# bytedance/monolith

Hardware: AMD Instinct MI355X
Metric: embedding lookups+updates/sec at 1B ids x dim64, Zipf(1.2) batch=65536 (higher is better)
Workload: dtype f32

## Files before the change

monolith_amd/_lib.py:

```python
import ctypes as C
import os
import subprocess

_DIR = os.path.dirname(os.path.abspath(__file__))
_SO = os.path.join(_DIR, "libmhte.so")
_SRC = os.path.join(_DIR, "csrc", "mhte.hip")
_DEPS = [_SRC] + sorted(os.path.join(_DIR, "csrc", h) for h in os.listdir(os.path.join(_DIR, "csrc"))
                        if h.endswith(".h")) + [os.path.join(_DIR, "..", "include", "monolith_amd_hash_table.h")]
_OVERRIDE = os.environ.get("MHTE_LIBRARY")

MHTE_OK = 0
MHTE_INVALID_ARGUMENT = 3
MHTE_NOT_FOUND = 5
MHTE_RESOURCE_EXHAUSTED = 8
MHTE_FAILED_PRECONDITION = 9
MHTE_INTERNAL = 13
MHTE_UNAVAILABLE = 14

MHTE_IDS_UNIQUE = 1
MHTE_SUM_DUPLICATES = 2
MHTE_EXACT_ORDER = 1
MHTE_DEFER_SLOWPATH = 2
MHTE_LAYOUT_ONE_FID_UNIQUE_ROWS = 1
ABI_VERSION = 19
# ... 71 lines not shown
def _stale():
  if not os.path.exists(_SO):
    return True
  if os.path.exists(_HASH_FILE):
    with open(_HASH_FILE) as f:
      return f.read().strip() != _source_hash()
  t = os.path.getmtime(_SO)
  return any(os.path.exists(d) and os.path.getmtime(d) > t for d in _DEPS)


def build_library(force=False, verbose=False):
  if not force and not _stale():
    _try_build_eager_loop(verbose)
    return _SO
  cmd = ["hipcc", "--offload-arch=gfx950", "-O3", "-std=c++17", "-ffp-contract=off", "-shared",
         "-fPIC", "-o", _SO, _SRC]
  if verbose:
    print(" ".join(cmd))
  if os.path.exists(_HASH_FILE):
    os.remove(_HASH_FILE)
  src_hash = _source_hash()
  subprocess.check_call(cmd)
  with open(_HASH_FILE, "w") as f:
    f.write(src_hash + "\n")
  _try_build_eager_loop(verbose)
  return _SO


_EAGER_SO = os.path.join(_DIR, "libmhte_eager.so")
_EAGER_SRC = os.path.join(_DIR, "csrc", "eager_loop.c")

# ... 184 lines not shown
```

monolith_amd/csrc/mhte.hip:

```cpp
#include <hip/hip_runtime.h>
#include <hip/hip_ext.h>
#include <hip/hip_fp16.h>

#include <algorithm>
#include <chrono>
#include <cstdio>
#include <cstdlib>
#include <cstring>
#include <memory>
#include <atomic>
#include <exception>
#include <mutex>
#include <future>
#include <thread>
#include <stdexcept>
#include <string>
#include <vector>

#include "../../include/monolith_amd_hash_table.h"
#include <unistd.h>
#include <dirent.h>
#include <ctype.h>

#include "mhte_ckpt.h"
// ... 419 lines not shown
    const uint32_t nb = (un + kDdBlock - 1) / kDdBlock;
    LAUNCH_HOT(kTagDedup, dd_insert_fast_kernel, nb, kDdBlock, st, d, ids, un, uids);
    LAUNCH_HOT(kTagDedup, dd_place_fast_kernel, nb, kDdBlock, st, d, un, inverse, lst_start, lst_end,
               seg_pos);
    const uint32_t nb_rank = (un + 1023) / 1024;
    const uint32_t hgrid = std::min<uint32_t>(256, un / (kLightMax + 1) + 1);
    LAUNCH_HOT(kTagDedup, dd_finish_kernel, nb_rank + hgrid, 1024, st, d, un, nb_rank, inverse,
               lst_start, lst_end, seg_pos, 0, n_unique_dev);
    hipError_t le = hipGetLastError();
    if (le != hipSuccess) {
      clean_cap = 0;
      HIP_OK(le);
    }
  }
};

struct Shape {
  int G;
  int VEC;
};
static Shape pick_shape(uint32_t dim, bool vec_ok) {
  Shape s;
  s.VEC = vec_ok ? 4 : 1;
  uint32_t units = (dim + s.VEC - 1) / s.VEC;
  uint32_t g = 8;
  while (g < units && g < 64) g <<= 1;
  s.G = int(g);
  return s;
}
static inline bool aligned16(const void* p) { return (reinterpret_cast<uintptr_t>(p) & 15u) == 0; }
// ... 572 lines not shown
    const uint32_t others = nxt.nblk + uint32_t(sp.enabled);
    const uint32_t slots = uint32_t(2 * num_cus);
    const uint32_t held = nxt.nblk;
    const uint32_t room = slots > held + 64 ? slots - held : 64u;
    auto blocks_for = [&](int unr) {
      const int64_t groups = (n + unr - 1) / unr;
      return uint32_t((groups * sh.G + kRdBlock - 1) / kRdBlock);
    };
    int unr = 2;
    while (unr < 3 && blocks_for(unr) > 2 * room) ++unr;
    const uint32_t nblk_l = std::min(blocks_for(unr), room);
    const dim3 grid(others + nblk_l);
    TableView v = view;
    v.trace = trace_region(kTagStepFwd, grid.x, kRdBlock);
    const bool basic = basic_opts();
#define CALLU(G_, V_, U_)                                                                        \
  do {                                                                                           \
    if (basic) {                                                                                 \
      LAUNCH_HOT(kTagStepFwd, (step_fwd_kernel<G_, V_, U_, true>), grid, kRdBlock, st, nxt, v, ids, n, out, \
                 count_hits ? 1 : 0, sp, nblk_l);                                                \
    } else {                                                                                     \
      LAUNCH_HOT(kTagStepFwd, (step_fwd_kernel<G_, V_, U_, false>), grid, kRdBlock, st, nxt, v, ids, n, out, \
                 count_hits ? 1 : 0, sp, nblk_l);                                                \
    }                                                                                            \
  } while (0)
#define CALL(G_, V_)                              \
  do {                                            \
    if (unr == 2) { CALLU(G_, V_, 2); }           \
    else { CALLU(G_, V_, 3); }                    \
  } while (0)
    DISPATCH_G_VEC(sh, CALL);
#undef CALL
#undef CALLU
    HIP_OK(hipGetLastError());
  }

  void step_backward(DedupWs& ws, DedupWs* ws_next, const int64_t* uids, int64_t n_max,
                     const uint32_t* n_dev, const float* grads, int64_t n, float* grad_u,
// ... 105 lines not shown
      da.ctr = ahead.ctr;
      da.ids = ahead.ids;
      da.cap_mask = ahead.cap_mask;
      da.n = ahead.n;
      da.nblk = ahead.nblk;
    }
    const dim3 grid(da.nblk + nblk_build + c.nblk_items + c.nblk_ids);
    TableView v = view;
    v.trace = trace_region(kTagStepBwd, grid.x, 256);
    const RunView cur = ws.rv;
    const bool basic = basic_opts();
    static const bool no_optk = getenv("MHTE_NO_OPTK") != nullptr;
    const bool filt = flt_slots != nullptr;
    const int optk =
        (!basic && nseg == 1 && sh.VEC == 4 && !view.seg[0].sr16 && !no_optk && !filt) ? int(view.seg[0].opt) : -1;
#define CALL_FILT(G_, V_, S_, F_)                                                                                \
  LAUNCH_HOT(kTagStepBwd, (step_bwd_kernel<G_, V_, S_, F_, -1, true>), grid, 256, st, nxt, nblk_build, v, cur, c, a, po, da)
#define CALL_OPTK(G_, K_)                                                                                     \
  LAUNCH_HOT(kTagStepBwd, (step_bwd_kernel<G_, 4, true, true, K_>), grid, 256, st, nxt, nblk_build, v, cur, c, a, po, da)
#define CALL(G_, V_) \
  do {                                                                                               \
    if (filt) {                                                                                      \
      if (basic && nseg == 1) CALL_FILT(G_, V_, true, false);                                        \
      else if (basic) CALL_FILT(G_, V_, false, false);                                               \
      else if (nseg == 1) CALL_FILT(G_, V_, true, true);                                             \
      else CALL_FILT(G_, V_, false, true);                                                           \
    } else if (V_ == 4 && optk == kOptMomentum) {                                                    \
      CALL_OPTK(G_, kOptMomentum);                                                                   \
    } else if (V_ == 4 && optk == kOptAdadelta) {                                                    \
      CALL_OPTK(G_, kOptAdadelta);                                                                   \
    } else if (V_ == 4 && optk == kOptRmsprop) {                                                     \
      CALL_OPTK(G_, kOptRmsprop);                                                                    \
    } else if (V_ == 4 && optk == kOptRmspropV2) {                                                   \
      CALL_OPTK(G_, kOptRmspropV2);                                                                  \
    } else if (V_ == 4 && optk == kOptAdam) {                                                        \
      CALL_OPTK(G_, kOptAdam);                                                                       \
    } else if (V_ == 4 && optk == kOptAmsgrad) {                                                     \
      CALL_OPTK(G_, kOptAmsgrad);                                                                    \
    } else if (!basic && nseg == 1) {                                                                \
      LAUNCH_HOT(kTagStepBwd, (step_bwd_kernel<G_, V_, true, true>), grid, 256, st, nxt, nblk_build, v, cur, c, a, po, da); \
    } else if (!basic) {                                                                             \
      LAUNCH_HOT(kTagStepBwd, (step_bwd_kernel<G_, V_, false, true>), grid, 256, st, nxt, nblk_build, v, cur, c, a, po, da); \
    } else if (nseg == 1) {                                                                          \
      LAUNCH_HOT(kTagStepBwd, (step_bwd_kernel<G_, V_, true>), grid, 256, st, nxt, nblk_build, v, cur, c, a, po, da);  \
    } else {                                                                                         \
      LAUNCH_HOT(kTagStepBwd, (step_bwd_kernel<G_, V_, false>), grid, 256, st, nxt, nblk_build, v, cur, c, a, po, da); \
    }                                                                                                \
  } while (0)
    DISPATCH_G_VEC(sh, CALL);
#undef CALL
#undef CALL_OPTK
#undef CALL_FILT
    hipError_t le = hipGetLastError();
    ws.r_stage = 0;
    if (nblk_build) {
      ws_next->r_stage = 2;
      ws_next->r_hints = true;
      ws_next->r_prealloc = reserve_next;
      ws_next->r_res_ctr = view.ctr;
      ws_next->r_res_serial = ctr_serial;
    }
    if (le != hipSuccess) {
      ws.r_clean_cap = 0;
      if (ws_next) ws_next->r_clean_cap = 0;
      HIP_OK(le);
    }
    filter_maintain(st, uint64_t(n));
// ... 3620 lines not shown
```

monolith_amd/csrc/mhte_step_kernels.h:

```cpp
#ifndef MHTE_STEP_KERNELS_H_
#define MHTE_STEP_KERNELS_H_

#include "mhte_kernels.h"

namespace mhte {

constexpr int kRdBlock = 1024;
constexpr int kRdLds = 2048;
constexpr int kRdStride = kRdLds + 1;
constexpr int kRdMaxBlocks = 64;
constexpr int kLongRun = kLightMax;
constexpr int kStepLightMax = 32;
constexpr int kMaxLongRuns = 16;
constexpr uint32_t kItemTarget = 256;
constexpr uint32_t kSpecSlackRows = 32;
#ifndef MHTE_BWD_OCC
#define MHTE_BWD_OCC 5
#endif
constexpr int kBwdBlocksPerCu = MHTE_BWD_OCC;

__device__ __forceinline__ void lds_barrier() {
  asm volatile("s_waitcnt lgkmcnt(0)\n\ts_barrier" ::: "memory");
}
__device__ __forceinline__ void lds_wave_sync() {
  asm volatile("s_waitcnt lgkmcnt(0)" ::: "memory");
}

__device__ __forceinline__ uint32_t run_pack(uint32_t first, uint32_t off, uint32_t cnt) {
  return (first << 21) | (off << 11) | cnt;
}
__device__ __forceinline__ uint32_t run_cnt(uint32_t v) { return v & 0x7ffu; }
__device__ __forceinline__ uint32_t run_off(uint32_t v) { return (v >> 11) & 0x3ffu; }
__device__ __forceinline__ uint32_t run_first(uint32_t v) { return v >> 21; }

// ... 39 lines not shown
  }
  if (i < 4) d.ctr[i] = 0;
}

struct RdLds {
  unsigned long long key[kRdStride];
  uint32_t cnt[kRdStride];
  uint32_t off[kRdStride];
  uint32_t first[kRdStride];
  uint16_t pos[kRdBlock];
  uint32_t wtot[16];
  uint32_t bm[kMaxLongRuns][32];
  uint32_t bmpre[kMaxLongRuns][32];
  uint8_t lslot[kRdStride + 3];
  uint32_t nlong;
};

__device__ __forceinline__ uint32_t rd_home(int64_t id) {
  return uint32_t(hash_key(id) >> 40) & (kRdLds - 1);
}

__device__ __forceinline__ void rd_dedup_role(const RunView& d, uint32_t bid, RdLds& L,
                                              WaveTrace& wt) {
  const uint32_t t = threadIdx.x;
  for (uint32_t i = t; i < uint32_t(kRdStride); i += kRdBlock) {
    L.key[i] = static_cast<unsigned long long>(kEmptyKey);
    L.cnt[i] = 0;
    L.lslot[i] = 0xff;
  }
  if (t < kMaxLongRuns * 32) (&L.bm[0][0])[t] = 0;
  if (t == 0) L.nlong = 0;
  if (bid == 0 && t < 4) d.ctr[t] = 0;
  const uint32_t p = bid * kRdBlock + t;
  const bool valid = p < d.n;
  const int64_t id = valid ? d.ids[p] : 0;
  lds_barrier();
  uint32_t ls = 0, arr = 0;
  if (valid) {
    if (id == kEmptyKey) {
      ls = kRdLds;
    } else {
      ls = rd_home(id);
      for (;;) {
        unsigned long long k = L.key[ls];
        if (k == static_cast<unsigned long long>(kEmptyKey)) {
          k = atomicCAS(&L.key[ls], static_cast<unsigned long long>(kEmptyKey),
                        static_cast<unsigned long long>(id));
          if (k == static_cast<unsigned long long>(kEmptyKey)) break;
        }
        if (k == static_cast<unsigned long long>(id)) break;
// ... 68 lines not shown
    const uint32_t c = L.cnt[ls], o = L.off[ls];
    uint32_t rank = 0;
    if (lsl != 0xffu) {
      rank = L.bmpre[lsl][t >> 5] + __popc(L.bm[lsl][t >> 5] & ((1u << (t & 31u)) - 1u));
    } else if (c > 1) {
      uint32_t i = 0;
      for (; i + 8 <= c; i += 8) {
        uint32_t x[8];
#pragma unroll
        for (int q = 0; q < 8; ++q) x[q] = L.pos[o + i + q];
#pragma unroll
        for (int q = 0; q < 8; ++q) rank += (x[q] < t) ? 1u : 0u;
      }
      for (; i < c; ++i) rank += (uint32_t(L.pos[o + i]) < t) ? 1u : 0u;
    }
    d.seg[bid * kRdBlock + o + rank] = uint16_t(t);
  }
  wt.mark(3);
  uint32_t lbase;
  if (speaker) {
    if (id != kEmptyKey) {
      while (cas_old != kEmptyKey && cas_old != id) {
        gs = (gs + 1u) & d.cap_mask;
        cas_old = static_cast<int64_t>(atomicCAS(reinterpret_cast<unsigned long long*>(&d.hs[gs].key),
                                                 static_cast<unsigned long long>(kEmptyKey),
                                                 static_cast<unsigned long long>(id)));
      }
    }
    lbase = uint32_t(atomicAdd(&d.hs[gs].cp, (static_cast<unsigned long long>(p) << 32) |
                                                 static_cast<unsigned long long>(L.cnt[ls])));
  }
  for (uint32_t i = t; i < uint32_t(kRdStride); i += kRdBlock) {
    d.btab_key[size_t(bid) * kRdStride + i] = static_cast<int64_t>(L.key[i]);
    d.btab_val[size_t(bid) * kRdStride + i] = run_pack(L.first[i] & 0x3ffu, L.off[i] & 0x3ffu, L.cnt[i]);
  }
  if (speaker) {
    const uint32_t c = L.cnt[ls];
    if (lbase + c <= uint32_t(kLightMax)) {
      const uint32_t o = L.off[ls];
      for (uint32_t i = 0; i < c; ++i)
        d.hlist[size_t(gs) * kLightMax + lbase + i] = bid * kRdBlock + uint32_t(L.pos[o + i]);
    }
  }
  wt.mark(4);
}

__global__ __launch_bounds__(kRdBlock) void rd_dedup_kernel(RunView d) {
  __shared__ RdLds L;
  WaveTrace wt(nullptr);
  rd_dedup_role(d, blockIdx.x, L, wt);
}

constexpr int kRd4Threads = 256;
constexpr int kRd4PerThread = kRdBlock / kRd4Threads;
struct __attribute__((aligned(16))) RdLds4 {
  unsigned long long key[kRdStride];
// ... 240 lines not shown
  return uint32_t(m < 0 ? m + int64_t(nshards) : m);
}
struct PackCtl {
  int64_t* send_ids;
  const unsigned long long* peer_win;
  unsigned long long peer_ids_off;
  uint32_t* slot_off;
  uint32_t* flags;
  uint32_t world, ids_block, rows_block;
  uint32_t hdr_word;
  uint32_t cap, id_off, row_off, dim;
};

__device__ __forceinline__ void rd_emit_items(const RunView& d, int64_t id, uint32_t hu, uint32_t c,
                                              uint32_t hrow, uint32_t hspec, unsigned long long hloc,
                                              int lane) {
  const uint32_t val = (uint32_t(lane) < d.nblk) ? rd_find_run_opt(d, uint32_t(lane), id) : 0u;
  const unsigned long long bm = __ballot(val != 0u);
  const uint32_t nbk = rd_item_blocks(c, d.item_target);
  const uint32_t b0 = uint32_t(lane) & ~(nbk - 1u);
  const unsigned long long rmask = (nbk == 64 ? ~0ull : ((1ull << nbk) - 1ull)) << b0;
  const bool leader = (uint32_t(lane) == b0) && (bm & rmask) != 0ull;
  const unsigned long long lm = __ballot(leader);
  const uint32_t nitems = __popcll(lm);
  uint32_t w0 = 0;
  if (lane == 0) w0 = atomicAdd(&d.ctr[2], nitems);
  w0 = __shfl(w0, 0);
  const uint32_t k = __popcll(lm & ((1ull << b0) - 1ull));
  if (leader) {
    ItemHdr hd;
    hd.id = id;
    hd.u = hu;
    hd.meta = b0 | (nbk << 8) | (k << 16) | (nitems << 24);
    hd.row = hrow;
    hd.spec = hspec;
    hd.loc = hloc;
    d.item_hdr[w0 + k] = hd;
  }
  if ((bm & rmask) != 0ull) d.item_runs[size_t(w0 + k) * 64 + (uint32_t(lane) - b0)] = val;
}

constexpr unsigned long long kNoLoc = ~0ull;
struct __attribute__((aligned(16))) URec {
  int64_t id;
  uint32_t cnt;
  uint32_t pos;
  uint32_t slot;
  uint32_t row;
  unsigned long long loc;
};
struct ProbeOut {
  URec* urec;
  uint32_t reserve;
};

template <bool PACK = false, bool PROBE = false>
__device__ __forceinline__ void rd_build_role(const RunView& d, uint32_t light_max, uint32_t bid,
                                              uint32_t nblocks, const PackCtl* pc = nullptr,
                                              const TableView* tv = nullptr, ProbeOut po = ProbeOut{}) {
  constexpr int Q = kBuildSlotsPerLane;
  __shared__ uint32_t sh_tot[4];
  __shared__ uint32_t sh_base;
  __shared__ uint32_t sh_mtot[PROBE ? 4 : 1];
  __shared__ uint32_t sh_mbase;
  __shared__ uint8_t sh_stage[PROBE ? 4 * 256 : 4];
  __shared__ uint32_t sh_pc[PACK ? kMaxShards : 1], sh_pb[PACK ? kMaxShards : 1];
  const uint32_t t = threadIdx.x;
  const int lane = t & 63;
  const uint32_t nslots = d.cap_mask + 2u;
  for (uint32_t bb = bid * (256u * Q); bb < nslots; bb += nblocks * (256u * Q)) {
    const uint32_t base = bb + (t >> 6) * (64u * Q);
    int64_t key[Q];
    uint32_t cnt[Q], pos[Q];
    unsigned long long occ[Q];
// ... 3 lines not shown
      lds_barrier();
    }
#pragma unroll
    for (int q = 0; q < Q; ++q) {
      const uint32_t sl = base + q * 64 + lane;
      const bool in = sl < nslots;
      const RdSlot sv = d.hs[in ? sl : 0u];
      key[q] = in ? sv.key : kEmptyKey;
      cnt[q] = in ? uint32_t(sv.cp) : 0u;
      pos[q] = in ? uint32_t(sv.cp >> 32) : 0u;
    }
#pragma unroll
    for (int q = 0; q < Q; ++q) {
      const uint32_t sl = base + q * 64 + lane;
      const bool o = key[q] != kEmptyKey;
      if (o) {
        d.hs[sl] = RdSlot{kEmptyKey, 0ull};
        if (sl == d.cap_mask + 1u) key[q] = kEmptyKey;
      }
      occ[q] = __ballot(o);
      total += uint32_t(__popcll(occ[q]));
    }
    uint32_t pown[Q], prank[Q];
    if (PACK) {
#pragma unroll
      for (int q = 0; q < Q; ++q) {
        pown[q] = prank[q] = 0;
        if ((occ[q] >> lane) & 1ull) {
          pown[q] = shard_of_id(key[q], pc->world);
          prank[q] = atomicAdd(&sh_pc[pown[q]], 1u);
        }
      }
    }
    if (lane == 0) sh_tot[t >> 6] = total;
// ... 122 lines not shown
          uint32_t m0 = sh_mbase;
          for (uint32_t w2 = 0; w2 < (t >> 6); ++w2) m0 += sh_mtot[w2];
          lds_barrier();
          if (miss) spec = m0 + uint32_t(__popcll(mm & ((1ull << lane) - 1ull)));
        }
        const unsigned long long floc = found ? (((fs & 4) ? i2 : i1) << 2) | uint64_t(fs & 3) : kNoLoc;
        const uint32_t frow = found ? fr : spec;
        if (have) {
          URec rec;
          rec.id = kid;
          rec.cnt = kc;
          rec.pos = kp;
          rec.slot = base + (src >> 6) * 64u + (src & 63u);
          rec.row = frow;
          rec.loc = floc;
          po.urec[kw0 + r] = rec;
        }
        unsigned long long hm = __ballot(have && kc > light_max);
        while (hm) {
          const int s2 = __ffsll(static_cast<long long>(hm)) - 1;
          hm &= hm - 1ull;
          const unsigned long long hl = __shfl(floc, s2);
          rd_emit_items(d, __shfl(kid, s2), kw0 + r0 + uint32_t(s2), __shfl(kc, s2),
                        hl != kNoLoc ? __shfl(frow, s2) : kNoRow, hl != kNoLoc ? kNoRow : __shfl(frow, s2),
                        hl != kNoLoc ? hl : 0ull, lane);
        }
      }
    }
  }
  if (t == 0) {
    if (atomicAdd(&d.ctr[1], 1u) == nblocks - 1) *d.n_unique = atomicAdd(&d.ctr[0], 0u);
  }
}

__global__ __launch_bounds__(256) void rd_build_kernel(RunView d, uint32_t light_max) {
  rd_build_role(d, light_max, blockIdx.x, gridDim.x);
}
__global__ __launch_bounds__(256) void rd_build_probe_kernel(RunView d, uint32_t light_max, TableView tv,
                                                             ProbeOut po) {
  rd_build_role<false, true>(d, light_max, blockIdx.x, gridDim.x, nullptr, &tv, po);
// ... 371 lines not shown
  out.deferred = deferred;
  return out;
}

struct ApplyLds {
  uint32_t pos[(256 / 8) * kStepLightMax];
  uint32_t rstart[65];
  uint32_t rval[64];
  float sum[256 * 4];
  uint32_t last;
};

template <int G, int VEC, bool ONESEG, bool HINT = false, bool FULL = false, int OPTK = -1, int FILT = -1>
__device__ __forceinline__ void rd_apply_role(const TableView& tv, const RunView& d,
                                              const ApplyCtl& c, const ApplyArgs& a, uint32_t bid,
                                              WaveTrace& wt, ApplyLds& L) {
  constexpr int WIN = G < 8 ? G : 8;
  constexpr int NG = 256 / G;
  const int lane = threadIdx.x & 63;
  const int j = lane & (G - 1);
  const int gbase = lane & ~(G - 1);
  const int grp = threadIdx.x / G;
  const uint32_t dim = tv.dim;
  const uint32_t e = uint32_t(j) * VEC;
  const bool ev = e < dim;

  if (bid >= c.nblk_items) {
    const uint32_t stride = c.nblk_ids * uint32_t(NG);
    const uint32_t k = bid - c.nblk_items;
    const uint32_t wave_s = __builtin_amdgcn_readfirstlane(threadIdx.x >> 6);
    uint32_t nu = c.n_max;
// ... 256 lines not shown
  for (uint32_t w = bid;; w += c.nblk_items) {
    const uint32_t nitems_all = d.ctr[2];
    const ItemHdr hd = d.item_hdr[w];
    const uint32_t rval = d.item_runs[size_t(w) * 64 + lane];
    asm volatile("" ::"v"(hd.meta), "v"(rval), "v"(nitems_all));
    if (w >= nitems_all) break;
    wt.mark(0);
    const uint32_t b0 = hd.meta & 0xffu, nbk = (hd.meta >> 8) & 0xffu, kk = (hd.meta >> 16) & 0xffu,
                   nitems = hd.meta >> 24;
    const bool ihint = hd.row != kNoRow;
    GBucket* const hb = global_bucket(tv.buckets + (hd.loc >> 2));
    int64_t vkey = hd.id;
    if (ihint && !c.trusted && threadIdx.x == 0) vkey = hb->key[hd.loc & 3ull];
    Probe<G> pr = probe_issue<G>(tv, hd.id, threadIdx.x < G && !ihint, j);
    const uint32_t reserved = threadIdx.x < G ? hd.spec : kNoRow;
    if (threadIdx.x < 64) {
      const uint32_t val = (uint32_t(lane) < nbk) ? rval : 0u;
      uint32_t incl = run_cnt(val);
#pragma unroll
      for (int o = 1; o < 64; o <<= 1) {
        const uint32_t v = __shfl_up(incl, o);
        if (lane >= o) incl += v;
      }
      sh_rval[lane] = val;
      sh_rstart[lane + 1] = incl;
      if (lane == 0) sh_rstart[0] = 0;
    }
    lds_barrier();
    wt.mark(1);
    const uint32_t E = c.pre_summed ? 0u : sh_rstart[64];
// ... 138 lines not shown
        sr.is_new = false;
        sr.deferred = false;
        if (valid && threadIdx.x == 0) hb->ts[hd.loc & 3ull] = vgpr_copy_of_uniform(a.ts);
      } else {
        sr = upsert_resolve<G>(tv, (Bucket*)pr.b, hd.id, valid, pr.k, pr.row, lane, vgpr_copy_of_uniform(a.ts),
                               reserved);
      }
      if (sr.deferred) {
        uint32_t ed = e;
#ifndef MHTE_NO_ANTIHOIST
        asm volatile("" : "+v"(ed));
#endif
        if (ev) tot.store(c.grad_u + int64_t(hd.u) * dim + ed);
        if (j == 0) defer_id(tv, c.pending, hd.u);
      } else if (valid) {
        if (FULL) optimize_row_reg_full<VEC, ONESEG, OPTK>(tv, row_ptr(tv, sr.r), sr.is_new, e, tot, a);
        else optimize_row_reg<VEC, ONESEG>(tv, row_ptr(tv, sr.r), sr.is_new, e, tot, a);
      }
    }
    wt.mark(4);
    lds_barrier();
  }
}

constexpr int kExactThreads = 512;
constexpr int kExactBufFloats = 16384;
constexpr int kExactMaxRows = 512;
struct __attribute__((aligned(16))) ExactLds {
  float buf[2][kExactBufFloats];
  uint32_t pos[3][kExactMaxRows];
  uint32_t rstart[65];
  uint32_t rbase[64];
// ... 137 lines not shown
__global__ __launch_bounds__(kExactThreads) void rd_exact_sum_kernel(RunView d, const float* __restrict__ grads,
                                                                     uint32_t dim, float* __restrict__ part) {
  __shared__ ExactLds L;
  rd_exact_sum_role<VEC>(d, grads, dim, ExactToPart{part, dim}, blockIdx.x, gridDim.x, L);
}

struct SlowArgs {
  const int64_t* uids;
  const float* grad_u;
  const uint32_t* pending;
  ApplyArgs a;
  int32_t enabled;
};


template <int G, int VEC, int UNR, bool BASIC = true>
__global__ __launch_bounds__(kRdBlock, 8) __attribute__((amdgpu_num_sgpr(80))) void step_fwd_kernel(RunView nxt, TableView tv,
                                                            const int64_t* __restrict__ ids,
                                                            int64_t n, float* __restrict__ out,
                                                            int count_hits, SlowArgs sp,
                                                            uint32_t nblk_l) {
  __shared__ __attribute__((aligned(16))) RdLds L;
  static_assert(sizeof(BfsSlot) * kMaxCuckooCount + sizeof(CuckooRecord) * kMaxBfsPathLen <=
                    sizeof(RdLds), "BFS scratch must fit the dedup's LDS");
  WaveTrace wt(tv.trace);
  uint32_t bid = blockIdx.x;
  if (bid < nxt.nblk) {
    rd_dedup_role(nxt, bid, L, wt);
    wt.end(3u);
    return;
  }
  bid -= nxt.nblk;
  if (sp.enabled) {
    if (bid == 0) {
      if (threadIdx.x < 64) {
        BfsSlot* q = reinterpret_cast<BfsSlot*>(&L);
        CuckooRecord* path = reinterpret_cast<CuckooRecord*>(q + kMaxCuckooCount);
        slowpath_role<VEC, kOpOptimize, false, true, BASIC>(tv, sp.uids, sp.grad_u, nullptr, nullptr, sp.a,
                                                            nullptr, sp.pending, q, path);
      }
      wt.end(4u);
      return;
    }
    bid -= 1;
  }
  const int64_t ngroups = (n + UNR - 1) / UNR;
  const uint32_t lbid = bid;
  const int64_t g_first = (int64_t(lbid) * kRdBlock + threadIdx.x) / G;
  int64_t id_first;
  {
    const int j = int(threadIdx.x & 63u) & (G - 1);
    const int64_t p0 = g_first * UNR + j;
    id_first = ids[(j < UNR && p0 < n) ? p0 : 0];
    if (!(j < UNR && p0 < n)) id_first = 0;
  }
  if (sp.enabled) {
    if (threadIdx.x == 0) {
      if (__hip_atomic_load(&tv.ctr->n_pending, __ATOMIC_RELAXED, __HIP_MEMORY_SCOPE_AGENT) != 0u) {
        while (__hip_atomic_load(&tv.ctr->n_pending, __ATOMIC_RELAXED, __HIP_MEMORY_SCOPE_AGENT) != 0u)
          __builtin_amdgcn_s_sleep(16);
        __builtin_amdgcn_fence(__ATOMIC_ACQUIRE, "agent");
      }
    }
    __syncthreads();
  }
  if (g_first < ngroups) lookup_role_u<G, VEC, UNR, 2>(tv, ids, n, nullptr, out, count_hits, g_first, &id_first);
#pragma unroll 1
  for (int64_t g = g_first + int64_t(nblk_l) * kRdBlock / G; g < ngroups;
       g += int64_t(nblk_l) * kRdBlock / G)
    lookup_role_u<G, VEC, UNR, 2>(tv, ids, n, nullptr, out, count_hits, g);
  wt.end(5u);
}

struct DedupArgs {
  RdSlot* hs;
  uint32_t* hlist;
  int64_t* btab_key;
  uint32_t* btab_val;
  uint16_t* seg;
  uint32_t* ctr;
  const int64_t* ids;
  uint32_t cap_mask, n;
  uint32_t nblk;
};

union __attribute__((aligned(16))) StepBwdLds {
  ApplyLds apply;
  RdLds4 dedup;
};
template <int G, int VEC, bool ONESEG, bool FULL = false, int OPTK = -1, bool FILT = false>
__global__ __launch_bounds__(256, kBwdBlocksPerCu) void step_bwd_kernel(RunView nxt, uint32_t nblk_build,
                                                       TableView tv, RunView cur, ApplyCtl c,
                                                       ApplyArgs a, ProbeOut po, DedupArgs da) {
  __shared__ StepBwdLds L;
  WaveTrace wt(tv.trace);
  uint32_t bid = blockIdx.x;
  if (bid < da.nblk) {
    RunView d{};
    d.hs = da.hs;
    d.hlist = da.hlist;
    d.btab_key = da.btab_key;
    d.btab_val = da.btab_val;
    d.seg = da.seg;
    d.ctr = da.ctr;
    d.ids = da.ids;
    d.cap_mask = da.cap_mask;
    d.n = da.n;
    d.nblk = da.nblk;
    rd_dedup4_role(d, bid, L.dedup);
    wt.end(3u);
    return;
  }
  bid -= da.nblk;
  if (bid < nblk_build) {
    rd_build_role<false, true>(nxt, uint32_t(kStepLightMax), bid, nblk_build, nullptr, &tv, po);
    wt.end(6u);
    return;
  }
  bid -= nblk_build;
  rd_apply_role<G, VEC, ONESEG, false, FULL, OPTK, FILT ? 1 : 0>(tv, cur, c, a, bid, wt, L.apply);
  wt.end(bid < c.nblk_items ? 7u : 8u);
}

struct GatherCtl {
  const float* in;
  float* out;
  const uint32_t* index;
  float* part;
  uint32_t* arrive;
  int64_t n_max;
  uint32_t dim;
  uint32_t nblk_items;
  uint32_t nblk_ids;
  uint32_t index_is_offset;
  const unsigned long long* peer_win;
  unsigned long long peer_out_off;
// ... 305 lines not shown
```

Measured before the change: 4.360 billion.

## Preload hot kernel args, add sc1 vector stores for dedup/build outputs, and prefetch rows

Enables AMDGPU kernel-argument preloading and reorders the fused step kernel signatures so the hot scalars (ids, counts, block splits, switch mask) come first and land in SGPRs. It also replaces scattered scalar stores of dedup directory, segment, hlist, item headers, urec and hash-slot resets with 16-byte global stores using the sc1 cache-policy bit, or relaxed atomic stores. The apply role gains an optional row prefetch into LDS. Each piece sits behind an environment switch, and there are no-preload kernel variants for comparison. The cost is more LDS per block, more code paths, and reliance on inline assembly and a compiler flag.

```diff
diff --git a/monolith_amd/_lib.py b/monolith_amd/_lib.py
--- a/monolith_amd/_lib.py
+++ b/monolith_amd/_lib.py
@@ -109,7 +109,7 @@
     _try_build_eager_loop(verbose)
     return _SO
   cmd = ["hipcc", "--offload-arch=gfx950", "-O3", "-std=c++17", "-ffp-contract=off", "-shared",
-         "-fPIC", "-o", _SO, _SRC]
+         "-fPIC", "-mllvm", "-amdgpu-kernarg-preload-count=16", "-o", _SO, _SRC]
   if verbose:
     print(" ".join(cmd))
   if os.path.exists(_HASH_FILE):
diff --git a/monolith_amd/csrc/mhte.hip b/monolith_amd/csrc/mhte.hip
--- a/monolith_amd/csrc/mhte.hip
+++ b/monolith_amd/csrc/mhte.hip
@@ -457,6 +457,24 @@
     }
   }
 };
+
+constexpr uint32_t kWtDefault = 1u | 2u | 8u | 16u | 32u;
+struct StepSwitches {
+  bool preload;
+  uint32_t sw;
+};
+static const StepSwitches& step_switches() {
+  static const StepSwitches v = [] {
+    StepSwitches r;
+    r.preload = getenv("MHTE_NO_PRELOAD") == nullptr;
+    r.sw = getenv("MHTE_NO_ITEM_PREFETCH") == nullptr ? kSwItemPf : 0u;
+    uint32_t wt = kWtDefault;
+    if (const char* e = getenv("MHTE_WT_STORES")) wt = uint32_t(atoi(e)) & 63u;
+    r.sw |= wt << 8;
+    return r;
+  }();
+  return v;
+}
 
 struct Shape {
   int G;
@@ -1059,14 +1077,25 @@
     TableView v = view;
     v.trace = trace_region(kTagStepFwd, grid.x, kRdBlock);
     const bool basic = basic_opts();
+    const StepSwitches& ss = step_switches();
+    const uint32_t sw = (ss.sw & (kSwWtDir | kSwWtSeg | kSwWtHlist)) | (v.trace ? kSwTrace : 0u);
+    const int32_t spe = sp.enabled;
 #define CALLU(G_, V_, U_)                                                                        \
   do {                                                                                           \
-    if (basic) {                                                                                 \
-      LAUNCH_HOT(kTagStepFwd, (step_fwd_kernel<G_, V_, U_, true>), grid, kRdBlock, st, nxt, v, ids, n, out, \
-                 count_hits ? 1 : 0, sp, nblk_l);                                                \
+    if (!ss.preload) {                                                                           \
+      if (basic) {                                                                               \
+        LAUNCH_HOT(kTagStepFwd, (step_fwd_kernel_np<G_, V_, U_, true>), grid, kRdBlock, st, nxt, ids, n, nxt.ids, \
+                   nxt.n, nxt.nblk, nblk_l, spe, sw, v, out, count_hits ? 1 : 0, sp);            \
+      } else {                                                                                   \
+        LAUNCH_HOT(kTagStepFwd, (step_fwd_kernel_np<G_, V_, U_, false>), grid, kRdBlock, st, nxt, ids, n, nxt.ids, \
+                   nxt.n, nxt.nblk, nblk_l, spe, sw, v, out, count_hits ? 1 : 0, sp);            \
+      }                                                                                          \
+    } else if (basic) {                                                                          \
+      LAUNCH_HOT(kTagStepFwd, (step_fwd_kernel<G_, V_, U_, true>), grid, kRdBlock, st, ids, n, nxt.ids, nxt.n, \
+                 nxt.nblk, nblk_l, spe, sw, nxt, v, out, count_hits ? 1 : 0, sp);                \
     } else {                                                                                     \
-      LAUNCH_HOT(kTagStepFwd, (step_fwd_kernel<G_, V_, U_, false>), grid, kRdBlock, st, nxt, v, ids, n, out, \
-                 count_hits ? 1 : 0, sp, nblk_l);                                                \
+      LAUNCH_HOT(kTagStepFwd, (step_fwd_kernel<G_, V_, U_, false>), grid, kRdBlock, st, ids, n, nxt.ids, nxt.n, \
+                 nxt.nblk, nblk_l, spe, sw, nxt, v, out, count_hits ? 1 : 0, sp);                \
     }                                                                                            \
   } while (0)
 #define CALL(G_, V_)                              \
@@ -1202,10 +1231,14 @@
     const bool filt = flt_slots != nullptr;
     const int optk =
         (!basic && nseg == 1 && sh.VEC == 4 && !view.seg[0].sr16 && !no_optk && !filt) ? int(view.seg[0].opt) : -1;
+    const StepSwitches& ss = step_switches();
+    const uint32_t sw = (ss.sw & (kSwItemPf | kSwWtReset | kSwWtUrec | kSwWtItems)) | (v.trace ? kSwTrace : 0u);
+#define BWD_LEAD cur.ctr, cur.item_hdr, cur.item_runs, c.urec, c.nblk_items, nblk_build, da.nblk, uint32_t(std::min<int64_t>(n_max, 0x7fffffff)), sw
+#define BWD_REST v, cur, c, a, po, da
 #define CALL_FILT(G_, V_, S_, F_)                                                                                \
-  LAUNCH_HOT(kTagStepBwd, (step_bwd_kernel<G_, V_, S_, F_, -1, true>), grid, 256, st, nxt, nblk_build, v, cur, c, a, po, da)
+  LAUNCH_HOT(kTagStepBwd, (step_bwd_kernel<G_, V_, S_, F_, -1, true>), grid, 256, st, BWD_LEAD, nxt, BWD_REST)
 #define CALL_OPTK(G_, K_)                                                                                     \
-  LAUNCH_HOT(kTagStepBwd, (step_bwd_kernel<G_, 4, true, true, K_>), grid, 256, st, nxt, nblk_build, v, cur, c, a, po, da)
+  LAUNCH_HOT(kTagStepBwd, (step_bwd_kernel<G_, 4, true, true, K_>), grid, 256, st, BWD_LEAD, nxt, BWD_REST)
 #define CALL(G_, V_) \
   do {                                                                                               \
     if (filt) {                                                                                      \
@@ -1226,19 +1259,25 @@
     } else if (V_ == 4 && optk == kOptAmsgrad) {                                                     \
       CALL_OPTK(G_, kOptAmsgrad);                                                                    \
     } else if (!basic && nseg == 1) {                                                                \
-      LAUNCH_HOT(kTagStepBwd, (step_bwd_kernel<G_, V_, true, true>), grid, 256, st, nxt, nblk_build, v, cur, c, a, po, da); \
+      LAUNCH_HOT(kTagStepBwd, (step_bwd_kernel<G_, V_, true, true>), grid, 256, st, BWD_LEAD, nxt, BWD_REST); \
     } else if (!basic) {                                                                             \
-      LAUNCH_HOT(kTagStepBwd, (step_bwd_kernel<G_, V_, false, true>), grid, 256, st, nxt, nblk_build, v, cur, c, a, po, da); \
+      LAUNCH_HOT(kTagStepBwd, (step_bwd_kernel<G_, V_, false, true>), grid, 256, st, BWD_LEAD, nxt, BWD_REST); \
+    } else if (!ss.preload && nseg == 1) {                                                           \
+      LAUNCH_HOT(kTagStepBwd, (step_bwd_kernel_np<G_, V_, true>), grid, 256, st, nxt, BWD_LEAD, BWD_REST); \
+    } else if (!ss.preload) {                                                                        \
+      LAUNCH_HOT(kTagStepBwd, (step_bwd_kernel_np<G_, V_, false>), grid, 256, st, nxt, BWD_LEAD, BWD_REST); \
     } else if (nseg == 1) {                                                                          \
-      LAUNCH_HOT(kTagStepBwd, (step_bwd_kernel<G_, V_, true>), grid, 256, st, nxt, nblk_build, v, cur, c, a, po, da);  \
+      LAUNCH_HOT(kTagStepBwd, (step_bwd_kernel<G_, V_, true>), grid, 256, st, BWD_LEAD, nxt, BWD_REST);  \
     } else {                                                                                         \
-      LAUNCH_HOT(kTagStepBwd, (step_bwd_kernel<G_, V_, false>), grid, 256, st, nxt, nblk_build, v, cur, c, a, po, da); \
+      LAUNCH_HOT(kTagStepBwd, (step_bwd_kernel<G_, V_, false>), grid, 256, st, BWD_LEAD, nxt, BWD_REST); \
     }                                                                                                \
   } while (0)
     DISPATCH_G_VEC(sh, CALL);
 #undef CALL
 #undef CALL_OPTK
 #undef CALL_FILT
+#undef BWD_LEAD
+#undef BWD_REST
     hipError_t le = hipGetLastError();
     ws.r_stage = 0;
     if (nblk_build) {
diff --git a/monolith_amd/csrc/mhte_step_kernels.h b/monolith_amd/csrc/mhte_step_kernels.h
--- a/monolith_amd/csrc/mhte_step_kernels.h
+++ b/monolith_amd/csrc/mhte_step_kernels.h
@@ -18,6 +18,20 @@
 #define MHTE_BWD_OCC 5
 #endif
 constexpr int kBwdBlocksPerCu = MHTE_BWD_OCC;
+
+constexpr uint32_t kSwItemPf = 1u;
+constexpr uint32_t kSwTrace = 2u;
+constexpr uint32_t kSwWtDir = 1u << 8;
+constexpr uint32_t kSwWtSeg = 1u << 9;
+constexpr uint32_t kSwWtHlist = 1u << 10;
+constexpr uint32_t kSwWtReset = 1u << 11;
+constexpr uint32_t kSwWtUrec = 1u << 12;
+constexpr uint32_t kSwWtItems = 1u << 13;
+
+typedef unsigned int wt_u32x4 __attribute__((ext_vector_type(4)));
+__device__ __forceinline__ void store_wt16(void* p, wt_u32x4 v) {
+  asm volatile("global_store_dwordx4 %0, %1, off sc1\n\ts_nop 1" ::"v"((MHTE_GLOBAL void*)p), "v"(v) : "memory");
+}
 
 __device__ __forceinline__ void lds_barrier() {
   asm volatile("s_waitcnt lgkmcnt(0)\n\ts_barrier" ::: "memory");
@@ -87,6 +101,7 @@
   uint32_t bmpre[kMaxLongRuns][32];
   uint8_t lslot[kRdStride + 3];
   uint32_t nlong;
+  uint16_t __attribute__((aligned(16))) segout[kRdBlock];
 };
 
 __device__ __forceinline__ uint32_t rd_home(int64_t id) {
@@ -94,7 +109,7 @@
 }
 
 __device__ __forceinline__ void rd_dedup_role(const RunView& d, uint32_t bid, RdLds& L,
-                                              WaveTrace& wt) {
+                                              WaveTrace& wt, uint32_t sw = 0) {
   const uint32_t t = threadIdx.x;
   for (uint32_t i = t; i < uint32_t(kRdStride); i += kRdBlock) {
     L.key[i] = static_cast<unsigned long long>(kEmptyKey);
@@ -103,10 +118,11 @@
   }
   if (t < kMaxLongRuns * 32) (&L.bm[0][0])[t] = 0;
   if (t == 0) L.nlong = 0;
-  if (bid == 0 && t < 4) d.ctr[t] = 0;
+  if ((sw & kSwWtSeg) && t < kRdBlock / 2) reinterpret_cast<uint32_t*>(L.segout)[t] = 0;
   const uint32_t p = bid * kRdBlock + t;
   const bool valid = p < d.n;
   const int64_t id = valid ? d.ids[p] : 0;
+  if (bid == 0 && t < 4) d.ctr[t] = 0;
   lds_barrier();
   uint32_t ls = 0, arr = 0;
   if (valid) {
@@ -205,7 +221,8 @@
       }
       for (; i < c; ++i) rank += (uint32_t(L.pos[o + i]) < t) ? 1u : 0u;
     }
-    d.seg[bid * kRdBlock + o + rank] = uint16_t(t);
+    if (sw & kSwWtSeg) L.segout[o + rank] = uint16_t(t);
+    else d.seg[bid * kRdBlock + o + rank] = uint16_t(t);
   }
   wt.mark(3);
   uint32_t lbase;
@@ -221,16 +238,59 @@
     lbase = uint32_t(atomicAdd(&d.hs[gs].cp, (static_cast<unsigned long long>(p) << 32) |
                                                  static_cast<unsigned long long>(L.cnt[ls])));
   }
-  for (uint32_t i = t; i < uint32_t(kRdStride); i += kRdBlock) {
-    d.btab_key[size_t(bid) * kRdStride + i] = static_cast<int64_t>(L.key[i]);
-    d.btab_val[size_t(bid) * kRdStride + i] = run_pack(L.first[i] & 0x3ffu, L.off[i] & 0x3ffu, L.cnt[i]);
+  if (sw & kSwWtSeg) {
+    lds_barrier();
+    if (t < kRdBlock / 8)
+      store_wt16(d.seg + bid * kRdBlock + 8u * t, *reinterpret_cast<const wt_u32x4*>(&L.segout[8u * t]));
+  }
+  if (sw & kSwWtDir) {
+    int64_t* const kt = d.btab_key + size_t(bid) * kRdStride;
+    uint32_t* const vt = d.btab_val + size_t(bid) * kRdStride;
+    const uint32_t kh = bid & 1u;
+    {
+      const uint32_t i = kh + 2u * t;
+      const unsigned long long k0 = L.key[i], k1 = L.key[i + 1];
+      wt_u32x4 v;
+      v.x = uint32_t(k0); v.y = uint32_t(k0 >> 32); v.z = uint32_t(k1); v.w = uint32_t(k1 >> 32);
+      store_wt16(kt + i, v);
+      if (t == 0) {
+        const uint32_t i1 = kh ? 0u : uint32_t(kRdLds);
+        __hip_atomic_store(reinterpret_cast<unsigned long long*>(kt + i1), L.key[i1], __ATOMIC_RELAXED,
+                           __HIP_MEMORY_SCOPE_AGENT);
+      }
+    }
+    const uint32_t vh = (4u - (bid & 3u)) & 3u;
+    const uint32_t nq = (uint32_t(kRdStride) - vh) / 4u;
+    auto val_of = [&](uint32_t i) { return run_pack(L.first[i] & 0x3ffu, L.off[i] & 0x3ffu, L.cnt[i]); };
+    if (t < nq) {
+      const uint32_t i = vh + 4u * t;
+      wt_u32x4 v;
+      v.x = val_of(i); v.y = val_of(i + 1); v.z = val_of(i + 2); v.w = val_of(i + 3);
+      store_wt16(vt + i, v);
+    } else if (t < nq + 8u) {
+      const uint32_t x = t - nq;
+      const uint32_t i = x < 3u ? x : vh + 4u * nq + (x - 3u);
+      if (x < 6u && (x < 3u ? x < vh : i < uint32_t(kRdStride)))
+        __hip_atomic_store(vt + i, val_of(i), __ATOMIC_RELAXED, __HIP_MEMORY_SCOPE_AGENT);
+    }
+  } else {
+    for (uint32_t i = t; i < uint32_t(kRdStride); i += kRdBlock) {
+      d.btab_key[size_t(bid) * kRdStride + i] = static_cast<int64_t>(L.key[i]);
+      d.btab_val[size_t(bid) * kRdStride + i] = run_pack(L.first[i] & 0x3ffu, L.off[i] & 0x3ffu, L.cnt[i]);
+    }
   }
   if (speaker) {
     const uint32_t c = L.cnt[ls];
     if (lbase + c <= uint32_t(kLightMax)) {
       const uint32_t o = L.off[ls];
-      for (uint32_t i = 0; i < c; ++i)
-        d.hlist[size_t(gs) * kLightMax + lbase + i] = bid * kRdBlock + uint32_t(L.pos[o + i]);
+      if (sw & kSwWtHlist) {
+        for (uint32_t i = 0; i < c; ++i)
+          __hip_atomic_store(&d.hlist[size_t(gs) * kLightMax + lbase + i], bid * kRdBlock + uint32_t(L.pos[o + i]),
+                             __ATOMIC_RELAXED, __HIP_MEMORY_SCOPE_AGENT);
+      } else {
+        for (uint32_t i = 0; i < c; ++i)
+          d.hlist[size_t(gs) * kLightMax + lbase + i] = bid * kRdBlock + uint32_t(L.pos[o + i]);
+      }
     }
   }
   wt.mark(4);
@@ -501,7 +561,7 @@
 
 __device__ __forceinline__ void rd_emit_items(const RunView& d, int64_t id, uint32_t hu, uint32_t c,
                                               uint32_t hrow, uint32_t hspec, unsigned long long hloc,
-                                              int lane) {
+                                              int lane, uint32_t sw = 0) {
   const uint32_t val = (uint32_t(lane) < d.nblk) ? rd_find_run_opt(d, uint32_t(lane), id) : 0u;
   const unsigned long long bm = __ballot(val != 0u);
   const uint32_t nbk = rd_item_blocks(c, d.item_target);
@@ -522,9 +582,21 @@
     hd.row = hrow;
     hd.spec = hspec;
     hd.loc = hloc;
-    d.item_hdr[w0 + k] = hd;
-  }
-  if ((bm & rmask) != 0ull) d.item_runs[size_t(w0 + k) * 64 + (uint32_t(lane) - b0)] = val;
+    if (sw & kSwWtItems) {
+      wt_u32x4 v0, v1;
+      v0.x = uint32_t(id); v0.y = uint32_t(uint64_t(id) >> 32); v0.z = hd.u; v0.w = hd.meta;
+      v1.x = hrow; v1.y = hspec; v1.z = uint32_t(hloc); v1.w = uint32_t(hloc >> 32);
+      store_wt16(&d.item_hdr[w0 + k], v0);
+      store_wt16(reinterpret_cast<char*>(&d.item_hdr[w0 + k]) + 16, v1);
+    } else {
+      d.item_hdr[w0 + k] = hd;
+    }
+  }
+  if ((bm & rmask) != 0ull) {
+    uint32_t* const rp = &d.item_runs[size_t(w0 + k) * 64 + (uint32_t(lane) - b0)];
+    if (sw & kSwWtItems) __hip_atomic_store(rp, val, __ATOMIC_RELAXED, __HIP_MEMORY_SCOPE_AGENT);
+    else *rp = val;
+  }
 }
 
 constexpr unsigned long long kNoLoc = ~0ull;
@@ -544,7 +616,8 @@
 template <bool PACK = false, bool PROBE = false>
 __device__ __forceinline__ void rd_build_role(const RunView& d, uint32_t light_max, uint32_t bid,
                                               uint32_t nblocks, const PackCtl* pc = nullptr,
-                                              const TableView* tv = nullptr, ProbeOut po = ProbeOut{}) {
+                                              const TableView* tv = nullptr, ProbeOut po = ProbeOut{},
+                                              uint32_t sw = 0) {
   constexpr int Q = kBuildSlotsPerLane;
   __shared__ uint32_t sh_tot[4];
   __shared__ uint32_t sh_base;
@@ -578,10 +651,18 @@
     for (int q = 0; q < Q; ++q) {
       const uint32_t sl = base + q * 64 + lane;
       const bool o = key[q] != kEmptyKey;
-      if (o) {
+      if (sw & kSwWtReset) {
+        if (sl < nslots) {
+          uint32_t z = 0;
+          asm volatile("" : "+v"(z));
+          wt_u32x4 v;
+          v.x = z | uint32_t(uint64_t(kEmptyKey)); v.y = z | uint32_t(uint64_t(kEmptyKey) >> 32); v.z = z; v.w = z;
+          store_wt16(&d.hs[sl], v);
+        }
+      } else if (o) {
         d.hs[sl] = RdSlot{kEmptyKey, 0ull};
-        if (sl == d.cap_mask + 1u) key[q] = kEmptyKey;
-      }
+      }
+      if (o && sl == d.cap_mask + 1u) key[q] = kEmptyKey;
       occ[q] = __ballot(o);
       total += uint32_t(__popcll(occ[q]));
     }
@@ -734,7 +815,15 @@
           rec.slot = base + (src >> 6) * 64u + (src & 63u);
           rec.row = frow;
           rec.loc = floc;
-          po.urec[kw0 + r] = rec;
+          if (sw & kSwWtUrec) {
+            wt_u32x4 v0, v1;
+            v0.x = uint32_t(kid); v0.y = uint32_t(uint64_t(kid) >> 32); v0.z = rec.cnt; v0.w = rec.pos;
+            v1.x = rec.slot; v1.y = frow; v1.z = uint32_t(floc); v1.w = uint32_t(floc >> 32);
+            store_wt16(&po.urec[kw0 + r], v0);
+            store_wt16(reinterpret_cast<char*>(&po.urec[kw0 + r]) + 16, v1);
+          } else {
+            po.urec[kw0 + r] = rec;
+          }
         }
         unsigned long long hm = __ballot(have && kc > light_max);
         while (hm) {
@@ -743,7 +832,7 @@
           const unsigned long long hl = __shfl(floc, s2);
           rd_emit_items(d, __shfl(kid, s2), kw0 + r0 + uint32_t(s2), __shfl(kc, s2),
                         hl != kNoLoc ? __shfl(frow, s2) : kNoRow, hl != kNoLoc ? kNoRow : __shfl(frow, s2),
-                        hl != kNoLoc ? hl : 0ull, lane);
+                        hl != kNoLoc ? hl : 0ull, lane, sw);
         }
       }
     }
@@ -1145,7 +1234,8 @@
 template <int G, int VEC, bool ONESEG, bool HINT = false, bool FULL = false, int OPTK = -1, int FILT = -1>
 __device__ __forceinline__ void rd_apply_role(const TableView& tv, const RunView& d,
                                               const ApplyCtl& c, const ApplyArgs& a, uint32_t bid,
-                                              WaveTrace& wt, ApplyLds& L) {
+                                              WaveTrace& wt, ApplyLds& L, uint32_t sw = 0,
+                                              float* rowpf = nullptr) {
   constexpr int WIN = G < 8 ? G : 8;
   constexpr int NG = 256 / G;
   const int lane = threadIdx.x & 63;
@@ -1432,6 +1522,26 @@
     if (ihint && !c.trusted && threadIdx.x == 0) vkey = hb->key[hd.loc & 3ull];
     Probe<G> pr = probe_issue<G>(tv, hd.id, threadIdx.x < G && !ihint, j);
     const uint32_t reserved = threadIdx.x < G ? hd.spec : kNoRow;
+    bool rowpf_on = false;
+    if constexpr (!FULL && ONESEG) {
+      rowpf_on = (sw & kSwItemPf) != 0u && rowpf != nullptr && ihint && !c.pre_summed &&
+                 (hd.row >> tv.chunk_shift) == 0u;
+      if (rowpf_on && threadIdx.x < G && ev) {
+        typedef const __attribute__((address_space(1))) void* pf_gptr;
+        typedef __attribute__((address_space(3))) void* pf_lptr;
+        const float* const rp0 = assume_global(tv.chunk0 + size_t(hd.row) * tv.row_floats);
+        const SegDesc sd0 = tv.seg[0];
+        const bool st1 = sd0.opt == kOptAdagrad || sd0.opt == kOptFtrl;
+        const float* const sp0 = rp0 + sd0.st_off + (e - sd0.w_off);
+        if constexpr (VEC == 4) {
+          __builtin_amdgcn_global_load_lds((pf_gptr)(rp0 + e), (pf_lptr)(rowpf), 16, 0, 0);
+          if (st1) __builtin_amdgcn_global_load_lds((pf_gptr)(sp0), (pf_lptr)(rowpf + 64 * VEC), 16, 0, 0);
+        } else {
+          __builtin_amdgcn_global_load_lds((pf_gptr)(rp0 + e), (pf_lptr)(rowpf), 4, 0, 0);
+          if (st1) __builtin_amdgcn_global_load_lds((pf_gptr)(sp0), (pf_lptr)(rowpf + 64 * VEC), 4, 0, 0);
+        }
+      }
+    }
     if (threadIdx.x < 64) {
       const uint32_t val = (uint32_t(lane) < nbk) ? rval : 0u;
       uint32_t incl = run_cnt(val);
@@ -1600,8 +1710,27 @@
         if (ev) tot.store(c.grad_u + int64_t(hd.u) * dim + ed);
         if (j == 0) defer_id(tv, c.pending, hd.u);
       } else if (valid) {
-        if (FULL) optimize_row_reg_full<VEC, ONESEG, OPTK>(tv, row_ptr(tv, sr.r), sr.is_new, e, tot, a);
-        else optimize_row_reg<VEC, ONESEG>(tv, row_ptr(tv, sr.r), sr.is_new, e, tot, a);
+        if constexpr (FULL) {
+          optimize_row_reg_full<VEC, ONESEG, OPTK>(tv, row_ptr(tv, sr.r), sr.is_new, e, tot, a);
+        } else if (ONESEG && rowpf_on && hok) {
+          asm volatile("s_waitcnt vmcnt(0)" ::: "memory");
+          RowRegs<VEC> rr;
+          vec_zero(rr.w);
+          vec_zero(rr.s1);
+          if (ev) {
+            const SegDesc sd0 = tv.seg[0];
+#pragma unroll
+            for (int cc = 0; cc < VEC; ++cc) rr.w.v[cc] = rowpf[lane * VEC + cc];
+            if (sd0.opt == kOptAdagrad || sd0.opt == kOptFtrl) {
+#pragma unroll
+              for (int cc = 0; cc < VEC; ++cc) rr.s1.v[cc] = rowpf[64 * VEC + lane * VEC + cc];
+            }
+          }
+          optimize_row_pre<VEC, ONESEG>(tv, assume_global(tv.chunk0 + size_t(hd.row) * tv.row_floats), false, e, tot, a,
+                                        rr);
+        } else {
+          optimize_row_reg<VEC, ONESEG>(tv, row_ptr(tv, sr.r), sr.is_new, e, tot, a);
+        }
       }
     }
     wt.mark(4);
@@ -1769,24 +1898,28 @@
 };
 
 
-template <int G, int VEC, int UNR, bool BASIC = true>
-__global__ __launch_bounds__(kRdBlock, 8) __attribute__((amdgpu_num_sgpr(80))) void step_fwd_kernel(RunView nxt, TableView tv,
-                                                            const int64_t* __restrict__ ids,
-                                                            int64_t n, float* __restrict__ out,
-                                                            int count_hits, SlowArgs sp,
-                                                            uint32_t nblk_l) {
+template <int G, int VEC, int UNR, bool BASIC>
+__device__ __forceinline__ void step_fwd_body(const int64_t* __restrict__ ids, int64_t n,
+                                              const int64_t* __restrict__ nxt_ids, uint32_t nxt_n,
+                                              uint32_t nxt_nblk, uint32_t nblk_l, int32_t sp_enabled, uint32_t sw,
+                                              const RunView& nxt_in, const TableView& tv, float* __restrict__ out,
+                                              int count_hits, const SlowArgs& sp) {
   __shared__ __attribute__((aligned(16))) RdLds L;
   static_assert(sizeof(BfsSlot) * kMaxCuckooCount + sizeof(CuckooRecord) * kMaxBfsPathLen <=
                     sizeof(RdLds), "BFS scratch must fit the dedup's LDS");
-  WaveTrace wt(tv.trace);
+  WaveTrace wt((sw & kSwTrace) ? tv.trace : nullptr);
   uint32_t bid = blockIdx.x;
-  if (bid < nxt.nblk) {
-    rd_dedup_role(nxt, bid, L, wt);
+  if (bid < nxt_nblk) {
+    RunView nxt = nxt_in;
+    nxt.ids = nxt_ids;
+    nxt.n = nxt_n;
+    nxt.nblk = nxt_nblk;
+    rd_dedup_role(nxt, bid, L, wt, sw);
     wt.end(3u);
     return;
   }
-  bid -= nxt.nblk;
-  if (sp.enabled) {
+  bid -= nxt_nblk;
+  if (sp_enabled) {
     if (bid == 0) {
       if (threadIdx.x < 64) {
         BfsSlot* q = reinterpret_cast<BfsSlot*>(&L);
@@ -1809,7 +1942,7 @@
     id_first = ids[(j < UNR && p0 < n) ? p0 : 0];
     if (!(j < UNR && p0 < n)) id_first = 0;
   }
-  if (sp.enabled) {
+  if (sp_enabled) {
     if (threadIdx.x == 0) {
       if (__hip_atomic_load(&tv.ctr->n_pending, __ATOMIC_RELAXED, __HIP_MEMORY_SCOPE_AGENT) != 0u) {
         while (__hip_atomic_load(&tv.ctr->n_pending, __ATOMIC_RELAXED, __HIP_MEMORY_SCOPE_AGENT) != 0u)
@@ -1825,6 +1958,23 @@
        g += int64_t(nblk_l) * kRdBlock / G)
     lookup_role_u<G, VEC, UNR, 2>(tv, ids, n, nullptr, out, count_hits, g);
   wt.end(5u);
+}
+
+template <int G, int VEC, int UNR, bool BASIC = true>
+__global__ __launch_bounds__(kRdBlock, 8) __attribute__((amdgpu_num_sgpr(80))) void step_fwd_kernel(
+    const int64_t* __restrict__ ids, int64_t n, const int64_t* __restrict__ nxt_ids, uint32_t nxt_n, uint32_t nxt_nblk,
+    uint32_t nblk_l, int32_t sp_enabled, uint32_t sw, RunView nxt, TableView tv, float* __restrict__ out,
+    int count_hits, SlowArgs sp) {
+  step_fwd_body<G, VEC, UNR, BASIC>(ids, n, nxt_ids, nxt_n, nxt_nblk, nblk_l, sp_enabled, sw, nxt, tv, out, count_hits,
+                                    sp);
+}
+template <int G, int VEC, int UNR, bool BASIC = true>
+__global__ __launch_bounds__(kRdBlock, 8) __attribute__((amdgpu_num_sgpr(80))) void step_fwd_kernel_np(
+    RunView nxt, const int64_t* __restrict__ ids, int64_t n, const int64_t* __restrict__ nxt_ids, uint32_t nxt_n,
+    uint32_t nxt_nblk, uint32_t nblk_l, int32_t sp_enabled, uint32_t sw, TableView tv, float* __restrict__ out,
+    int count_hits, SlowArgs sp) {
+  step_fwd_body<G, VEC, UNR, BASIC>(ids, n, nxt_ids, nxt_n, nxt_nblk, nblk_l, sp_enabled, sw, nxt, tv, out, count_hits,
+                                    sp);
 }
 
 struct DedupArgs {
@@ -1840,17 +1990,22 @@
 };
 
 union __attribute__((aligned(16))) StepBwdLds {
-  ApplyLds apply;
+  struct {
+    ApplyLds apply;
+    float __attribute__((aligned(16))) rowpf[2 * 64 * 4];
+  } a;
   RdLds4 dedup;
 };
-template <int G, int VEC, bool ONESEG, bool FULL = false, int OPTK = -1, bool FILT = false>
-__global__ __launch_bounds__(256, kBwdBlocksPerCu) void step_bwd_kernel(RunView nxt, uint32_t nblk_build,
-                                                       TableView tv, RunView cur, ApplyCtl c,
-                                                       ApplyArgs a, ProbeOut po, DedupArgs da) {
+template <int G, int VEC, bool ONESEG, bool FULL, int OPTK, bool FILT>
+__device__ __forceinline__ void step_bwd_body(uint32_t* ctr, ItemHdr* item_hdr, uint32_t* item_runs, const URec* urec,
+                                              uint32_t nblk_items, uint32_t nblk_build, uint32_t da_nblk,
+                                              uint32_t n_max, uint32_t sw, const RunView& nxt, const TableView& tv,
+                                              const RunView& cur_in, const ApplyCtl& c_in, const ApplyArgs& a,
+                                              const ProbeOut& po, const DedupArgs& da) {
   __shared__ StepBwdLds L;
-  WaveTrace wt(tv.trace);
+  WaveTrace wt((sw & kSwTrace) ? tv.trace : nullptr);
   uint32_t bid = blockIdx.x;
-  if (bid < da.nblk) {
+  if (bid < da_nblk) {
     RunView d{};
     d.hs = da.hs;
     d.hlist = da.hlist;
@@ -1861,20 +2016,45 @@
     d.ids = da.ids;
     d.cap_mask = da.cap_mask;
     d.n = da.n;
-    d.nblk = da.nblk;
+    d.nblk = da_nblk;
     rd_dedup4_role(d, bid, L.dedup);
     wt.end(3u);
     return;
   }
-  bid -= da.nblk;
+  bid -= da_nblk;
   if (bid < nblk_build) {
-    rd_build_role<false, true>(nxt, uint32_t(kStepLightMax), bid, nblk_build, nullptr, &tv, po);
+    rd_build_role<false, true>(nxt, uint32_t(kStepLightMax), bid, nblk_build, nullptr, &tv, po, sw);
     wt.end(6u);
     return;
   }
   bid -= nblk_build;
-  rd_apply_role<G, VEC, ONESEG, false, FULL, OPTK, FILT ? 1 : 0>(tv, cur, c, a, bid, wt, L.apply);
-  wt.end(bid < c.nblk_items ? 7u : 8u);
+  RunView cur = cur_in;
+  cur.ctr = ctr;
+  cur.item_hdr = item_hdr;
+  cur.item_runs = item_runs;
+  ApplyCtl c = c_in;
+  c.urec = urec;
+  c.nblk_items = nblk_items;
+  c.n_max = int64_t(n_max);
+  rd_apply_role<G, VEC, ONESEG, false, FULL, OPTK, FILT ? 1 : 0>(tv, cur, c, a, bid, wt, L.a.apply, sw, L.a.rowpf);
+  wt.end(bid < nblk_items ? 7u : 8u);
+}
+
+template <int G, int VEC, bool ONESEG, bool FULL = false, int OPTK = -1, bool FILT = false>
+__global__ __launch_bounds__(256, kBwdBlocksPerCu) void step_bwd_kernel(
+    uint32_t* ctr, ItemHdr* item_hdr, uint32_t* item_runs, const URec* urec, uint32_t nblk_items, uint32_t nblk_build,
+    uint32_t da_nblk, uint32_t n_max, uint32_t sw, RunView nxt, TableView tv, RunView cur, ApplyCtl c, ApplyArgs a,
+    ProbeOut po, DedupArgs da) {
+  step_bwd_body<G, VEC, ONESEG, FULL, OPTK, FILT>(ctr, item_hdr, item_runs, urec, nblk_items, nblk_build, da_nblk, n_max,
+                                                  sw, nxt, tv, cur, c, a, po, da);
+}
+template <int G, int VEC, bool ONESEG>
+__global__ __launch_bounds__(256, kBwdBlocksPerCu) void step_bwd_kernel_np(
+    RunView nxt, uint32_t* ctr, ItemHdr* item_hdr, uint32_t* item_runs, const URec* urec, uint32_t nblk_items,
+    uint32_t nblk_build, uint32_t da_nblk, uint32_t n_max, uint32_t sw, TableView tv, RunView cur, ApplyCtl c,
+    ApplyArgs a, ProbeOut po, DedupArgs da) {
+  step_bwd_body<G, VEC, ONESEG, false, -1, false>(ctr, item_hdr, item_runs, urec, nblk_items, nblk_build, da_nblk, n_max,
+                                                  sw, nxt, tv, cur, c, a, po, da);
 }
 
 struct GatherCtl {
```

Result: no change. 4.332 billion (-0.6%).
